# paschalidoud/raynet

Hardware: AMD Instinct MI355X
Metric: rays/sec (whole node) at 5 views x 64 depths x 128^3 voxels (higher is better)
Workload: dtype f32

## Files before the change

include/raynet_hip.h:

```cpp
#ifndef RAYNET_HIP_H
#define RAYNET_HIP_H

#include <stdint.h>

#ifdef __cplusplus
extern "C" {
#endif

typedef enum {
    RN_OK = 0,
    RN_ERR_INVALID = -1,
    RN_ERR_HIP = -2,
    RN_ERR_NO_DEVICE = -3,
    RN_ERR_STATE = -4
} rn_status;

typedef struct {
    int32_t M;
    int32_t D;
    int32_t N;
    int32_t F;
    int32_t H;
    int32_t W;
    int32_t padding;
// ... 160 lines not shown
    RN_RUN_DEPTH_RANGE = 16
} rn_run_phase;
int rn_scene_run(rn_ctx *ctx, const rn_scene_plan *plan, int32_t phases, int32_t iteration,
                 int32_t image, void *stream);

int rn_stitch_rows(rn_ctx *ctx, int64_t n, const float *rows, const int32_t *index, float *out,
                   void *stream);

typedef enum {
    RN_K_TRAVERSE = 1,
    RN_K_SWEEP_MAP = 2,
    RN_K_BP = 3,
    RN_K_DEPTH = 4,
    RN_K_ACC = 5,
    RN_K_OTHER = 6,
    RN_K_SCATTER = 7
} rn_kernel_id;
int rn_prof_begin(rn_ctx *ctx, int32_t capacity);
int rn_prof_select(rn_ctx *ctx, uint32_t kernel_mask);
int rn_prof_end(rn_ctx *ctx, int32_t *count, int32_t *kernel_ids_host, int32_t *n_rays_host,
                float *ms_host);
int rn_prof_offsets(rn_ctx *ctx, float *start_ms_host);

int rn_selftest_arith(rn_ctx *ctx, int32_t n, const float *a, float *out, void *stream);
int rn_selftest_quotient(rn_ctx *ctx, int32_t n, const float *x, const float *d, float *out,
                         void *stream);

int rn_selftest_feature_offsets(rn_ctx *ctx, int32_t n, const float *P, const float *ray_start,
                                const float *ray_end, int32_t *out, void *stream);

int rn_selftest_mapping(rn_ctx *ctx, int32_t n, const float *a, const float *b, const float *t,
                        float *out, void *stream);


int rn_plane_weights(rn_ctx *ctx, int32_t n, const int32_t *rvi, const int32_t *rvc,
                     const float *ray_start, const float *ray_end, int32_t *left, float *c1,
                     float *c2, void *stream);

int rn_train_bp_sweep(rn_ctx *ctx, int32_t n, const float *Sr, const int32_t *rvi,
                      const int32_t *rvc, const float *acc_in, const float *msgs_in,
                      float *acc_out, float *msgs_out, void *stream);
int rn_train_depth(rn_ctx *ctx, int32_t n, const float *Sr, const int32_t *rvi,
                   const int32_t *rvc, const float *acc, const float *msgs, float *S_new,
                   void *stream);

int rn_train_bp_sweep_bwd(rn_ctx *ctx, int32_t n, const float *Sr, const int32_t *rvi,
                          const int32_t *rvc, const float *acc_in, const float *msgs_in,
                          const float *g_msgs_out, const float *g_acc_out, float *g_Sr,
                          float *g_acc_in, float *g_msgs_in, void *stream);

int rn_train_depth_bwd(rn_ctx *ctx, int32_t n, const float *Sr, const int32_t *rvi,
                       const int32_t *rvc, const float *acc, const float *msgs,
                       const float *g_S_new, float *g_Sr, float *g_acc, float *g_msgs,
                       void *stream);


int rn_depthmap_points(rn_ctx *ctx, int32_t H, int32_t W, const double *P_pinv,
                       const double *camera_center, const float *depth_map, double *points,
                       void *stream);

int rn_consistency_tau(rn_ctx *ctx, int32_t n, int32_t H, int32_t W, int32_t first,
                       const double *points, const double *P, const double *camera_center,
                       const float *depth_map, double *tau, void *stream);

int rn_nearest_neighbors(rn_ctx *ctx, int32_t n_ref, const float *ref_xyzw, int32_t n_query,
                         const float *query_xyzw, float *dist, int32_t *idx, void *stream);
// ... 47 lines not shown
```

raynet_amd/_lib.py:

```python
import ctypes
import os
import subprocess

_HERE = os.path.dirname(os.path.abspath(__file__))
CSRC = os.path.join(_HERE, "csrc")
ENV_LIB = os.environ.get("RAYNET_HIP_LIB") or None
LIB_PATH = ENV_LIB or os.path.join(CSRC, "libraynet_hip.so")
HEADER = os.path.join(os.path.dirname(_HERE), "include", "raynet_hip.h")

HIPCC_FLAGS = [
    "--offload-arch=gfx950", "-O3", "-std=c++17",
    "-ffp-contract=off",
    "-munsafe-fp-atomics",
    "-Wno-unused-value", "-fPIC", "-shared",
]

RN_OK = 0
STATUS = {0: "RN_OK", -1: "RN_ERR_INVALID", -2: "RN_ERR_HIP", -3: "RN_ERR_NO_DEVICE",
          -4: "RN_ERR_STATE"}


class RaynetHipError(RuntimeError):
    pass

# ... 108 lines not shown
    "rn_scene_bp_sweep_fixed": [_P, _I, _P, _P, _P, _P, _P, _P, _I, _I, _P],
    "rn_acc_combine_fixed": [_P, _P, _F, _P, _P],
    "rn_acc_combine_fixed_range": [_P, _P, _L, _F, _P, _P],
    "rn_acc_combine": [_P, _P, _F, _P, _P],
    "rn_acc_reduce_local": [_P, _P, _P, _P],
    "rn_acc_add_prior": [_P, _P, _F, _P],
    "rn_scene_depth": [_P, _I, _P, _P, _P, _P, _P, _P, _I, _P, _P, _P],
    "rn_prof_begin": [_P, _I],
    "rn_prof_select": [_P, ctypes.c_uint32],
    "rn_prof_end": [_P, ctypes.POINTER(_I), _P, _P, _P],
    "rn_plane_weights": [_P, _I, _P, _P, _P, _P, _P, _P, _P, _P],
    "rn_train_bp_sweep": [_P, _I, _P, _P, _P, _P, _P, _P, _P, _P],
    "rn_train_depth": [_P, _I, _P, _P, _P, _P, _P, _P, _P],
    "rn_train_bp_sweep_bwd": [_P, _I] + [_P] * 11,
    "rn_train_depth_bwd": [_P, _I] + [_P] * 10,
    "rn_depthmap_points": [_P, _I, _I, _P, _P, _P, _P, _P],
    "rn_consistency_tau": [_P, _I, _I, _I, _I, _P, _P, _P, _P, _P, _P],
    "rn_nearest_neighbors": [_P, _I, _P, _I, _P, _P, _P, _P],
    "rn_mesh_keys": [_P, _I, _P, _P, _P, _P],
    "rn_mesh_build": [_P, _I, _P, _P, _P, _P, _P, ctypes.POINTER(_I), _P],
    "rn_mesh_raycast": [_P, _I, _P, _P, _P, _P, _P, _P, _P],
    "rn_mesh_depthmap": [_P, _I, _I, _P, _P, _P, _P, _P, _P],
    "rn_mesh_closest": [_P, _I, _P, _P, _P, _P, _P, _P, _P],
    "rn_mesh_areas": [_P, _I, _P, _P, _P],
    "rn_mesh_sample": [_P, _I, _I, _P, _P, _L, _P, _P, _P],
    "rn_voxel_mask": [_P, _I, _P, _P, _I, _I, _I, _P, _P, _P],
    "rn_thin_keys": [_P, _I, _P, _D, _D, _D, _D, _L, _P, _P, _P, _P],
    "rn_thin_round": [_P, _I, _P, _I, _P, _P, _P, _P, _D, _P, _P, _P],
    "rn_prof_offsets": [_P, _P],
    "rn_selftest_arith": [_P, _I, _P, _P, _P],
    "rn_selftest_quotient": [_P, _I, _P, _P, _P, _P],
    "rn_selftest_mapping": [_P, _I, _P, _P, _P, _P, _P],
    "rn_selftest_feature_offsets": [_P, _I, _P, _P, _P, _P, _P],
    "rn_timer_start": [_P, _P],
    "rn_timer_stop": [_P, _P, ctypes.POINTER(_F)],
}

_lib = None


def load():
    global _lib
    if _lib is not None:
        return _lib
    if not os.path.exists(LIB_PATH):
        raise RaynetHipError(
            "%s is missing: run `python -c 'import __graft_entry__ as g; g.build()'` "
            "(raynet_amd has no CPU fallback)" % LIB_PATH)
    import torch
    lib = ctypes.CDLL(LIB_PATH)
    for name, argtypes in SIGNATURES.items():
        fn = getattr(lib, name)
        fn.argtypes = argtypes
        fn.restype = ctypes.c_int
    lib.rn_destroy.restype = None
    lib.rn_last_error.restype = ctypes.c_char_p
    lib.rn_version.restype = ctypes.c_char_p
    lib.rn_acc_size.restype = ctypes.c_int64
    lib.rn_slab_boxes_size.restype = ctypes.c_int64
    _lib = lib
    return lib
```

raynet_amd/csrc/raynet_hip.hip:

```cpp
#include "raynet_kernels.h"

#include <cstdarg>
#include <cstdio>
#include <cstdlib>
#include <iterator>
#include <type_traits>
#include <utility>
#include <vector>

#include "../../include/raynet_hip.h"
#include "raynet_box_policy.h"

using namespace rn;

namespace {

constexpr int BLOCK = 256;
constexpr int RAY_BLOCK = 256;
constexpr int WAVES_PER_BLOCK = BLOCK / WAVE;
constexpr int SWEEP_BLOCK = 256;
constexpr int SWEEP_WAVES = SWEEP_BLOCK / WAVE;
constexpr int NXCD = 8;

constexpr int XCD_CHUNK_SWEEP = 2048 * 64 / 256;
// ... 66 lines not shown
__global__ __launch_bounds__(BLOCK) void k_selftest_arith(int n, const float *__restrict__ a,
                                                          float *out) {
    const int i = blockIdx.x * BLOCK + threadIdx.x;
    if (i >= n) return;
    out[i] = roundf(a[i]);
    out[(size_t)n + i] = round_half_away(a[i]);
}
__global__ __launch_bounds__(BLOCK) void k_selftest_quotient(int n, const float *__restrict__ x,
                                                             const float *__restrict__ d,
                                                             float *out) {
    const int i = blockIdx.x * BLOCK + threadIdx.x;
    if (i >= n) return;
    bool sure;
    const float rd = __builtin_amdgcn_rcpf(d[i]);
    const float fast = round_quotient_fast(x[i], rd, sure);
    sure = sure && reciprocal_is_normal(rd);
    out[i] = round_half_away(x[i] / d[i]);
    out[(size_t)n + i] = fast;
    out[2 * (size_t)n + i] = sure ? 1.0f : 0.0f;
}
__global__ __launch_bounds__(BLOCK) void k_selftest_offsets(Params p, int n,
                                                            const float *__restrict__ P,
                                                            const float *__restrict__ starts,
                                                            const float *__restrict__ ends,
                                                            int32_t *out) {
    int lane;
    const int r = ray_of_wave(n, lane);
    if (r < 0) return;
    float s[3], e[3];
    for (int i = 0; i < 3; i++) {
        s[i] = starts[3 * r + i];
        e[i] = ends[3 * r + i];
    }
    const float pad_shift = (float)(p.padding - (p.padding - 1) / 2);
    for (int base = 0; base < p.D; base += WAVE) {
        const int k = min(base + lane, p.D - 1);
        float point[3];
        plane_point(s, e, k, p.D, point);
        for (int v = 0; v < p.N; v++) {
            const int generic = feature_offset(p, P + 12 * v, point) / p.F;
            const int coop = feature_offset_bytes<7>(p, P + 12 * v, point, pad_shift) >> 7;
            if (base + lane < p.D) {
                int32_t *o = out + (((size_t)r * p.N + v) * p.D + k) * 2;
                o[0] = generic;
                o[1] = coop;
            }
        }
    }
}
__global__ __launch_bounds__(BLOCK) void k_selftest_mapping(Params p, int n,
                                                            const float *__restrict__ a,
                                                            const float *__restrict__ b,
                                                            const float *__restrict__ t,
                                                            float *out) {
    extern __shared__ float pos[];
    for (int i = threadIdx.x; i <= p.D; i += BLOCK) pos[i] = 0.0f + i * p.plane_step;
    __syncthreads();
    const int i = blockIdx.x * BLOCK + threadIdx.x;
    if (i >= n) return;
    const float y = 1.0f / b[i];
    out[i] = a[i] / b[i];
    out[(size_t)n + i] = markstein_div(a[i], b[i], y);
    out[2 * (size_t)n + i] = markstein_ok(b[i]) && markstein_ok_dividend(a[i]) ? 1.0f : 0.0f;
    const float tc = clampf(t[i], 1e-4f, 1 - 1e-4f);
    out[3 * (size_t)n + i] = (float)plane_index_walk(tc, p.D, p.plane_step);
    out[4 * (size_t)n + i] = (float)plane_index_from_table(pos, tc, p.D);
}
template <bool TO_GRID>
__global__ void k_acc_regrid(Params p, const float *__restrict__ src, float *dst) {
    const int64_t G = (int64_t)p.gx * p.gy * p.gz;
    for (int64_t i = blockIdx.x * (int64_t)blockDim.x + threadIdx.x; i < G;
         i += (int64_t)gridDim.x * blockDim.x) {
        const int z = (int)(i % p.gz), y = (int)((i / p.gz) % p.gy), x = (int)(i / ((int64_t)p.gz * p.gy));
        const int64_t b = ((((int64_t)(x >> 2) * p.nby + (y >> 2)) * p.nbz + (z >> 2)) << 6) |
                          ((x & 3) << 4) | ((y & 3) << 2) | (z & 3);
        if (TO_GRID) dst[i] = src[b];
        else dst[b] = src[i];
    }
}
__global__ void k_stitch_rows(int64_t n, const float *__restrict__ rows,
                              const int32_t *__restrict__ index, float *out) {
    const int64_t n4 = n >> 2;
    for (int64_t i = blockIdx.x * (int64_t)blockDim.x + threadIdx.x; i < n4;
         i += (int64_t)gridDim.x * blockDim.x) {
        const int4 ix = reinterpret_cast<const int4 *>(index)[i];
        reinterpret_cast<float4 *>(out)[i] = make_float4(rows[ix.x], rows[ix.y], rows[ix.z], rows[ix.w]);
    }
    if (blockIdx.x == 0 && threadIdx.x < (n & 3)) {
        const int64_t i = (n4 << 2) + threadIdx.x;
        out[i] = rows[index[i]];
    }
}
__global__ void k_add_scalar(float *a, int64_t n, float v) {
    for (int64_t i = blockIdx.x * (int64_t)blockDim.x + threadIdx.x; i < n;
         i += (int64_t)gridDim.x * blockDim.x)
        a[i] = v + a[i];
}

#include "raynet_prepare.inl"
// ... 798 lines not shown
    RN_OPEN(ctx, n, all_set(a, out));
    hipLaunchKernelGGL(k_selftest_arith, dim3(thread_blocks(n)), dim3(BLOCK), 0, S(stream), n, a, out);
    RN_LAUNCH_CHECK(ctx);
    return RN_OK;
}

int rn_selftest_quotient(rn_ctx *ctx, int32_t n, const float *x, const float *d, float *out,
                         void *stream) {
    RN_OPEN(ctx, n, all_set(x, d, out));
    hipLaunchKernelGGL(k_selftest_quotient, dim3(thread_blocks(n)), dim3(BLOCK), 0, S(stream), n, x,
                       d, out);
    RN_LAUNCH_CHECK(ctx);
    return RN_OK;
}

int rn_selftest_feature_offsets(rn_ctx *ctx, int32_t n, const float *P, const float *ray_start,
                                const float *ray_end, int32_t *out, void *stream) {
    RN_OPEN(ctx, n, all_set(P, ray_start, ray_end, out));
    hipLaunchKernelGGL(k_selftest_offsets, dim3(ray_blocks(n)), dim3(BLOCK), 0, S(stream), ctx->p, n,
                       P, ray_start, ray_end, out);
    RN_LAUNCH_CHECK(ctx);
    return RN_OK;
}

int rn_selftest_mapping(rn_ctx *ctx, int32_t n, const float *a, const float *b, const float *t,
                        float *out, void *stream) {
    RN_OPEN(ctx, n, all_set(a, b, t, out));
    hipLaunchKernelGGL(k_selftest_mapping, dim3(thread_blocks(n)), dim3(BLOCK),
                       sizeof(float) * (ctx->p.D + 1), S(stream), ctx->p, n, a, b, t, out);
    RN_LAUNCH_CHECK(ctx);
    return RN_OK;
}

int rn_prof_offsets(rn_ctx *ctx, float *start_ms_host) {
    if (!ctx || !start_ms_host) return fail(ctx, RN_ERR_INVALID, "bad argument");
    for (int i = 0; i < ctx->prof_n; i++)
        RN_HIP(ctx, hipEventElapsedTime(start_ms_host + i, ctx->prof_ev[0], ctx->prof_ev[2 * i]));
    return RN_OK;
}


int rn_timer_start(rn_ctx *ctx, void *stream) {
    if (!ctx) return RN_ERR_INVALID;
    RN_HIP(ctx, hipEventRecord(ctx->ev0, S(stream)));
    return RN_OK;
}

int rn_timer_stop(rn_ctx *ctx, void *stream, float *ms_out) {
    if (!ctx || !ms_out) return RN_ERR_INVALID;
    RN_HIP(ctx, hipEventRecord(ctx->ev1, S(stream)));
    RN_HIP(ctx, hipEventSynchronize(ctx->ev1));
    RN_HIP(ctx, hipEventElapsedTime(ms_out, ctx->ev0, ctx->ev1));
    return RN_OK;
}

}

#include "raynet_train.inl"

#include "raynet_eval.inl"

#include "raynet_mesh.inl"

#include "raynet_filters.inl"
```

raynet_amd/csrc/raynet_kernels.h:

```cpp
#pragma once
#include <hip/hip_runtime.h>
#include <float.h>
#include <stdint.h>

namespace rn {

constexpr int WAVE = 64;
constexpr int MAX_VIEWS = 16;

typedef float float2v __attribute__((ext_vector_type(2)));
typedef float float4v __attribute__((ext_vector_type(4)));

struct Params {
    int M, D, N, F, H, W, padding;
    int gx, gy, gz;
    int nby, nbz;
    int Hf, Wf;
    float plane_step;
    float bbox[6];
};

struct FeatureViews {
    const float *v[MAX_VIEWS];
};
// ... 55 lines not shown
__device__ __forceinline__ float wave_sum(float x) {
    RN_WAVE_REDUCE("v_add_f32_dpp", x);
    return lane63(x);
}
__device__ __forceinline__ float wave_max(float x) {
    RN_WAVE_REDUCE("v_max_f32_dpp", x);
    return lane63(x);
}
__device__ __forceinline__ int wave_max_i(int x) {
    RN_WAVE_REDUCE("v_max_i32_dpp", x);
    return lane63i(x);
}
__device__ __forceinline__ int wave_min_i(int x) {
    RN_WAVE_REDUCE("v_min_i32_dpp", x);
    return lane63i(x);
}
__device__ __forceinline__ int uniform(int x) { return __builtin_amdgcn_readfirstlane(x); }
__device__ __forceinline__ void wave_sync() {
    __builtin_amdgcn_fence(__ATOMIC_ACQ_REL, "wavefront");
    __builtin_amdgcn_wave_barrier();
}

__device__ __forceinline__ float clampf(float x, float a, float b) {
    return __builtin_amdgcn_fmed3f(x, a, b);
}

__device__ __forceinline__ float round_half_away(float x) {
    return __builtin_truncf(x + __builtin_copysignf(0x1.fffffep-2f, x));
}

__device__ __forceinline__ bool reciprocal_is_normal(float rcp_n) {
    return __builtin_amdgcn_classf(rcp_n, 0x108);
}
__device__ __forceinline__ float round_quotient_fast(float x, float rcp_n, bool &sure) {
    const float q = x * rcp_n;
    const float r = __builtin_rintf(q);
    sure = __builtin_fabsf(q - r) < __builtin_fmaf(__builtin_fabsf(q), -0x1p-21f, 0.5f);
    return r;
}

__device__ __forceinline__ void sample_in_bbox(const Params &p, int ray_idx,
                                               const float *__restrict__ P_inv,
                                               const float *__restrict__ cc, float s[3],
                                               float e[3]) {
    const float px = (float)(ray_idx / p.H);
    const float py = (float)(ray_idx % p.H);
    double o[4];
#pragma unroll
    for (int r = 0; r < 4; r++) {
        double a = 0.0;
        a += (double)(P_inv[3 * r + 0] * px);
        a += (double)(P_inv[3 * r + 1] * py);
        a += (double)P_inv[3 * r + 2] * 1.0;
        o[r] = a;
    }
    float dir[3];
#pragma unroll
    for (int i = 0; i < 3; i++) dir[i] = (float)(o[i] / o[3] - (double)cc[i]);
    float t_near = -INFINITY, t_far = INFINITY;
#pragma unroll
    for (int i = 0; i < 3; i++) {
        const float t1 = (float)(((double)p.bbox[i] - (double)cc[i]) / (double)dir[i]);
        const float t2 = (float)(((double)p.bbox[3 + i] - (double)cc[i]) / (double)dir[i]);
        t_near = fmaxf(fminf(t1, t2), t_near);
        t_far = fminf(fmaxf(t1, t2), t_far);
    }
    const float near_mask = (fabsf(t_near) < fabsf(t_far)) ? 1.0f : 0.0f;
    const float tn = t_near * near_mask + t_far * (1 - near_mask);
    const float tf = (1 - near_mask) * t_near + near_mask * t_far;
#pragma unroll
    for (int i = 0; i < 3; i++) {
        s[i] = cc[i] + tn * dir[i];
        e[i] = cc[i] + tf * dir[i];
    }
}

__device__ __forceinline__ int feature_offset(const Params &p, const float *__restrict__ Pv,
                                              const float point[3]) {
    float x = 0.0f, y = 0.0f, n = 0.0f;
    x += Pv[0] * point[0]; x += Pv[1] * point[1]; x += Pv[2] * point[2]; x += Pv[3] * 1;
    y += Pv[4] * point[0]; y += Pv[5] * point[1]; y += Pv[6] * point[2]; y += Pv[7] * 1;
    n += Pv[8] * point[0]; n += Pv[9] * point[1]; n += Pv[10] * point[2]; n += Pv[11] * 1;
    x = x / n;
    y = y / n;
    const int half = (p.padding - 1) / 2;
    int fx = (int)(roundf(x) + p.padding - half);
    int fy = (int)(roundf(y) + p.padding - half);
    fx = min(max(fx, 0), p.W);
    fy = min(max(fy, 0), p.H);
    if (fx == 0 || fy == 0) fx = fy = 0;
    return (fy * p.Wf + fx) * p.F;
}

__device__ __forceinline__ void project_fast(const float *__restrict__ Pv, const float point[3],
                                             float &x, float &y, float &n, float &rx, float &ry,
                                             unsigned long long &sure) {
    x = Pv[0] * point[0]; y = Pv[4] * point[0]; n = 0.0f;
    x += Pv[1] * point[1]; x += Pv[2] * point[2]; x += Pv[3] * 1;
    y += Pv[5] * point[1]; y += Pv[6] * point[2]; y += Pv[7] * 1;
    n += Pv[8] * point[0]; n += Pv[9] * point[1]; n += Pv[10] * point[2]; n += Pv[11] * 1;
    const float rn = __builtin_amdgcn_rcpf(n);
    bool sure_x, sure_y;
    rx = round_quotient_fast(x, rn, sure_x);
    ry = round_quotient_fast(y, rn, sure_y);
    unsigned long long normal_rcp;
    asm("v_cmp_class_f32_e64 %0, %1, %2" : "=s"(normal_rcp) : "v"(rn), "v"(0x108));
    sure = __builtin_amdgcn_ballot_w64(sure_x) & __builtin_amdgcn_ballot_w64(sure_y) & normal_rcp;
}
__device__ __forceinline__ void project_ieee(float x, float y, float n, float &rx, float &ry) {
    rx = round_half_away(x / n);
    ry = round_half_away(y / n);
}
template <int LOG2_VEC_BYTES>
__device__ __forceinline__ int project_offset(const Params &p, float rx, float ry, float pad_shift) {
    rx += pad_shift;
    ry += pad_shift;
    const unsigned fx = (unsigned)(int)__builtin_amdgcn_fmed3f(rx, 0.0f, (float)p.W);
    const unsigned fy = (unsigned)(int)__builtin_amdgcn_fmed3f(ry, 0.0f, (float)p.H);
    const unsigned off = (__umul24(fy, (unsigned)p.Wf) + fx) << LOG2_VEC_BYTES;
    return min(fx, fy) == 0u ? 0 : (int)off;
}
template <int LOG2_VEC_BYTES>
__device__ __forceinline__ int feature_offset_bytes(const Params &p,
                                                    const float *__restrict__ Pv,
                                                    const float point[3], float pad_shift) {
    float x, y, n, rx, ry;
    unsigned long long sure;
    project_fast(Pv, point, x, y, n, rx, ry, sure);
    if (sure != __builtin_amdgcn_read_exec())
        project_ieee(x, y, n, rx, ry);
    return project_offset<LOG2_VEC_BYTES>(p, rx, ry, pad_shift);
}

__device__ __forceinline__ void plane_point(const float s[3], const float e[3], int k, int D,
                                            float point[3]) {
#pragma unroll
    for (int a = 0; a < 3; a++) point[a] = s[a] + k * (e[a] - s[a]) / (D - 1);
}

__device__ __forceinline__ void sweep_generic(const Params &p, const FeatureViews &fv,
                                              const float *const *__restrict__ tbl,
                                              const float *__restrict__ P, const float s[3],
                                              const float e[3], int lane, float *Sl) {
    const int pairs = (p.N * (p.N - 1)) / 2;
    for (int base = 0; base < p.D; base += WAVE) {
        const int k = base + lane;
        if (k < p.D) {
            float point[3];
            plane_point(s, e, k, p.D, point);
            float acc = 0.0f;
            for (int i = 0; i < p.N; i++) {
                const float *fi = (tbl ? tbl[i] : fv.v[i]) + feature_offset(p, P + 12 * i, point);
                for (int j = i + 1; j < p.N; j++) {
                    const float *fj =
                        (tbl ? tbl[j] : fv.v[j]) + feature_offset(p, P + 12 * j, point);
                    float dot = 0.0f;
                    for (int f = 0; f < p.F; f++) dot += fi[f] * fj[f];
                    acc += dot;
                }
            }
            Sl[k] = acc / pairs;
        }
    }
}

constexpr int SWEEP_V4 = 1;
constexpr int SWEEP_UNROLL2_MAX_VIEWS = 6;
#define RN_ADD_DPP(OUT, MOVED, STAY, CTRL)                                                   \
    asm("s_nop 1\n\tv_add_f32_dpp %0, %1, %2 " CTRL " row_mask:0xf bank_mask:0xf"           \
        : "=v"(OUT) : "v"(MOVED), "v"(STAY))
#define RN_DPP_XOR1 "quad_perm:[1,0,3,2]"
#define RN_DPP_XOR2 "quad_perm:[2,3,0,1]"
#define RN_DPP_MIRROR8 "row_half_mirror"

template <int NV, int V4, bool REF_HELD = false>
__device__ __forceinline__ float sweep_round(const float *const (&vbase)[NV], const int (&offb)[NV],
                                             int src, unsigned part_bytes,
                                             const float2v (&ref)[2 * V4]) {
    float2v f2[NV][2 * V4];
#pragma unroll
    for (int v = 0; v < NV; v++) {
        if (REF_HELD && v == 0) {
#pragma unroll
            for (int c = 0; c < 2 * V4; c++) f2[0][c] = ref[c];
            continue;
        }
        const unsigned ob = (unsigned)__shfl(offb[v], src) + part_bytes;
        typedef const __attribute__((address_space(1))) char *gptr;
        typedef const __attribute__((address_space(1))) float4v *gptr4;
#pragma unroll
        for (int q = 0; q < V4; q++) {
            const float4v f = *(gptr4)((gptr)vbase[v] + ob + 16u * q);
            f2[v][2 * q] = float2v{f.x, f.y};
            f2[v][2 * q + 1] = float2v{f.z, f.w};
        }
    }
    float acc;
    {
#pragma clang fp contract(fast)
        float2v run[2 * V4], a2[2 * V4];
#pragma unroll
        for (int c = 0; c < 2 * V4; c++) {
            run[c] = f2[0][c];
            a2[c] = float2v{0.f, 0.f};
        }
#pragma unroll
        for (int j = 1; j < NV; j++) {
#pragma unroll
            for (int c = 0; c < 2 * V4; c++) {
                a2[c] = run[c] * f2[j][c] + a2[c];
                if (j + 1 < NV) run[c] += f2[j][c];
            }
        }
        float2v t = a2[0];
#pragma unroll
        for (int c = 1; c < 2 * V4; c++) t += a2[c];
        acc = t.x + t.y;
    }
    return acc;
}

template <int NV, int LPS, int V4, bool REF_HELD, int RPW, bool PARTIAL>
__device__ __forceinline__ float sweep_rounds(const float *const (&vbase)[NV], const int (&offb)[NV],
                                              int sub, int part, unsigned part_bytes,
                                              const float2v (&ref)[RPW][2 * V4], int live, int nrays,
                                              int &mine_round) {
    constexpr int SPL = WAVE / LPS;
    constexpr int DPAD = WAVE / RPW;
    static_assert(DPAD % (2 * SPL) == 0 || LPS != 8, "a pair of load rounds stays within one ray");
    float mine = 0.0f;
    if (LPS == 8 && NV <= SWEEP_UNROLL2_MAX_VIEWS) {
        const bool odd = (part ^ (part >> 2)) & 1;
        mine_round = (part & ~1) | (int)odd;
#pragma unroll
        for (int t = 0; t < LPS / 2; t++) {
            const int first = (2 * t) * SPL;
            if (PARTIAL && (first % DPAD >= live || first / DPAD >= nrays)) continue;
            const float2v(&rf)[2 * V4] = ref[RPW == 1 ? 0 : first / DPAD];
            const float a0 = sweep_round<NV, V4, REF_HELD>(vbase, offb, first + sub, part_bytes, rf);
            const float a1 = sweep_round<NV, V4, REF_HELD>(vbase, offb, first + SPL + sub, part_bytes, rf);
            const float stay = odd ? a1 : a0, moved = odd ? a0 : a1;
            float r;
            RN_ADD_DPP(r, moved, stay, RN_DPP_XOR1);
            RN_ADD_DPP(r, r, r, RN_DPP_XOR2);
            RN_ADD_DPP(r, r, r, RN_DPP_MIRROR8);
            if ((part >> 1) == t) mine = r;
        }
    } else {
        static_assert(LPS <= 8, "sweep_coop folds at most 8 lanes per plane");
        mine_round = part;
#pragma unroll
        for (int it = 0; it < LPS; it++) {
            const int first = it * SPL;
            if (PARTIAL && (first % DPAD >= live || first / DPAD >= nrays)) continue;
            float acc = sweep_round<NV, V4, REF_HELD>(vbase, offb, first + sub, part_bytes,
                                                      ref[RPW == 1 ? 0 : first / DPAD]);
            if (LPS >= 2) RN_ADD_DPP(acc, acc, acc, RN_DPP_XOR1);
            if (LPS >= 4) RN_ADD_DPP(acc, acc, acc, RN_DPP_XOR2);
            if (LPS >= 8) RN_ADD_DPP(acc, acc, acc, RN_DPP_MIRROR8);
            if (part == it) mine = acc;
        }
    }
    return mine;
}

template <int NV, int LPS, bool FAST = false, int RPW = 1>
__device__ __forceinline__ void sweep_coop(const Params &p, const FeatureViews &fv,
                                           const float *const *__restrict__ tbl,
                                           const float *__restrict__ P, const float s[3],
                                           const float e[3], int lane, float *Sl, int nrays = 1) {
    constexpr int SPL = WAVE / LPS;
    constexpr int V4 = SWEEP_V4;
    constexpr int DPAD = WAVE / RPW;
    const float *vbase[NV];
#pragma unroll
    for (int v = 0; v < NV; v++) vbase[v] = tbl ? tbl[v] : fv.v[v];
    const int sub = lane / LPS;
    const int part = lane % LPS;
    const unsigned part_bytes = (16u * V4) * (unsigned)part;
    const int pairs = (NV * (NV - 1)) / 2;
    constexpr int LOG2_VEC_BYTES = LPS * V4 == 8 ? 7 : LPS * V4 == 4 ? 6 : LPS * V4 == 2 ? 5 : 4;
    static_assert((16 * V4 * LPS) == (1 << LOG2_VEC_BYTES), "vector bytes must be a power of two");
    const float pad_shift = (float)(p.padding - (p.padding - 1) / 2);
    const int q_lane = RPW == 1 ? 0 : lane / DPAD;
    for (int base = 0; base < (RPW == 1 ? p.D : 1); base += WAVE) {
        int offb[NV];
        {
            const int k = min(RPW == 1 ? base + lane : lane % DPAD, p.D - 1);
            float point[3];
            plane_point(s, e, k, p.D, point);
#pragma unroll
            for (int v = 0; v < NV; v++)
                offb[v] = feature_offset_bytes<LOG2_VEC_BYTES>(p, P + 12 * v, point, pad_shift);
        }
        int off0[RPW];
#pragma unroll
        for (int q = 0; q < RPW; q++) off0[q] = __builtin_amdgcn_readlane(offb[0], q * DPAD);
        int off0_mine = off0[0];
#pragma unroll
        for (int q = 1; q < RPW; q++) off0_mine = q_lane == q ? off0[q] : off0_mine;
        const bool ref_held = __all(offb[0] == off0_mine);
        float2v ref[RPW][2 * V4];
#pragma unroll
        for (int q = 0; q < RPW; q++)
#pragma unroll
            for (int c = 0; c < 2 * V4; c++) ref[q][c] = float2v{0.f, 0.f};
        if (ref_held) {
            typedef const __attribute__((address_space(1))) char *gptr;
            typedef const __attribute__((address_space(1))) float4v *gptr4;
#pragma unroll
            for (int q = 0; q < RPW; q++)
#pragma unroll
                for (int c = 0; c < V4; c++) {
                    const float4v f = *(gptr4)((gptr)vbase[0] + (unsigned)off0[q] + part_bytes + 16u * c);
                    ref[q][2 * c] = float2v{f.x, f.y};
                    ref[q][2 * c + 1] = float2v{f.z, f.w};
                }
        }
        float mine = 0.0f;
        int mine_round;
        const int live = RPW == 1 ? p.D - base : p.D;
        const bool full = live >= DPAD && nrays == RPW;
        if (ref_held && full)
            mine = sweep_rounds<NV, LPS, V4, true, RPW, false>(vbase, offb, sub, part, part_bytes, ref, live, nrays, mine_round);
        else if (ref_held)
            mine = sweep_rounds<NV, LPS, V4, true, RPW, true>(vbase, offb, sub, part, part_bytes, ref, live, nrays, mine_round);
        else
            mine = sweep_rounds<NV, LPS, V4, false, RPW, true>(vbase, offb, sub, part, part_bytes, ref, live, nrays, mine_round);
        const int j = mine_round * SPL + sub;
        const int k = RPW == 1 ? base + j : j % DPAD;
        const int q = RPW == 1 ? 0 : j / DPAD;
        if (k < p.D && q < nrays) Sl[q * p.D + k] = FAST ? mine * (1.0f / pairs) : mine / pairs;
    }
}

#define RN_GROUP_REDUCE16(OP, X)                                                 \
    RN_SCAN_STEP(OP, X, "quad_perm:[1,0,3,2] row_mask:0xf bank_mask:0xf");       \
    RN_SCAN_STEP(OP, X, "quad_perm:[2,3,0,1] row_mask:0xf bank_mask:0xf");       \
    RN_SCAN_STEP(OP, X, "row_half_mirror row_mask:0xf bank_mask:0xf");           \
// ... 6 lines not shown
    return lane < 32 ? lo : hi;
}
template <int G>
__device__ __forceinline__ float group_max(float x, int lane) {
    static_assert(G == 16 || G == 32, "groups of 16 or 32 lanes");
    RN_GROUP_REDUCE16("v_max_f32_dpp", x);
    if (G == 32) RN_SCAN_STEP("v_max_f32_dpp", x, "row_bcast:15 row_mask:0xa bank_mask:0xf");
    return group_pick<G>(x, lane);
}
template <int G>
__device__ __forceinline__ float group_sum(float x, int lane) {
    static_assert(G == 16 || G == 32, "groups of 16 or 32 lanes");
    RN_GROUP_REDUCE16("v_add_f32_dpp", x);
    if (G == 32) RN_SCAN_STEP("v_add_f32_dpp", x, "row_bcast:15 row_mask:0xa bank_mask:0xf");
    return group_pick<G>(x, lane);
}

template <bool FAST>
__device__ __forceinline__ float vdiv(float a, float b) {
    return FAST ? a * __builtin_amdgcn_rcpf(b) : a / b;
}
__device__ __forceinline__ float exp_nonpos(float x) {
    const float log2e_hi = 0x1.715476p+0f, log2e_lo = 0x1.4ae0bep-26f;
    const float ph = x * log2e_hi;
    float pl = __builtin_fmaf(x, log2e_hi, -ph);
    pl = __builtin_fmaf(x, log2e_lo, pl);
    const float e = __builtin_rintf(ph);
    const float a = (ph - e) + pl;
    const float r = __builtin_amdgcn_ldexpf(__builtin_amdgcn_exp2f(a), (int)e);
    return x < -0x1.9d1da00000000p+6f ? 0.0f : r;
}
template <bool FAST = false>
__device__ __forceinline__ void softmax_column(int D, int lane, float *Sl) {
    float mx = -INFINITY;
    for (int k = lane; k < D; k += WAVE) mx = fmaxf(mx, Sl[k]);
    mx = wave_max(mx);
    float sum = 0.0f;
    for (int k = lane; k < D; k += WAVE) {
        const float d = Sl[k] - mx;
#if !defined(RN_EXACT_OCC_EXP) && !defined(RN_EXACT_SOFTMAX_EXP)
        const float v = FAST ? __builtin_amdgcn_exp2f(d * 0x1.715476p+0f)
                             : (d <= 0.0f ? exp_nonpos(d) : expf(d));
#else
        const float v = d <= 0.0f ? exp_nonpos(d) : expf(d);
#endif
        Sl[k] = v;
        sum += v;
    }
    sum = wave_sum(sum);
    for (int k = lane; k < D; k += WAVE) Sl[k] = vdiv<FAST>(Sl[k], sum);
}

template <bool FAST, int RPW>
__device__ __forceinline__ void softmax_columns(int D, int lane, float *Sl) {
    constexpr int DPAD = WAVE / RPW;
    const int k = lane % DPAD;
    float *x = Sl + (lane / DPAD) * D + k;
    const bool mine = k < D;
    const float mx = group_max<DPAD>(mine ? *x : -INFINITY, lane);
    float v = 0.0f;
    if (mine) {
        const float d = *x - mx;
#if !defined(RN_EXACT_OCC_EXP) && !defined(RN_EXACT_SOFTMAX_EXP)
        v = FAST ? __builtin_amdgcn_exp2f(d * 0x1.715476p+0f) : (d <= 0.0f ? exp_nonpos(d) : expf(d));
#else
        v = d <= 0.0f ? exp_nonpos(d) : expf(d);
// ... 17 lines not shown
        z = row[3 * i + 2];
    }
}
__device__ __forceinline__ int pack_voxel(int x, int y, int z) {
    return (x << 20) | (y << 10) | z;
}

constexpr int SLAB_BOX_STEPS = 16;
__host__ __device__ __forceinline__ int slab_box_count(int M) {
    return (M + SLAB_BOX_STEPS - 1) / SLAB_BOX_STEPS;
}

__device__ __forceinline__ float markstein_div(float a, float b, float y) {
    const float q0 = a * y;
    const float r = __builtin_fmaf(-b, q0, a);
    return __builtin_fmaf(r, y, q0);
}
__device__ __forceinline__ bool markstein_ok(float b) {
    return b >= 0x1p-60f && b <= 0x1p60f;
}
__device__ __forceinline__ bool markstein_ok_dividend(float a) {
    return __builtin_fabsf(a) < 0x1p60f;
}
__device__ __forceinline__ int plane_index_from_table(const float *pos, float t, int D) {
    const int a = max((int)(t * (D - 1)), 1);
    return (a - 1) + (pos[a] < t ? 1 : 0) + (pos[a + 1] < t ? 1 : 0);
}
__device__ __forceinline__ int plane_index_walk(float t, int D, float step) {
    int L = max(0, (int)(t * (D - 1)) - 1);
    while ((t - (0.0f + L * step) > 0) && (t - (0.0f + (L + 1) * step) > 0)) L++;
    return L;
}

template <bool PACKED, bool FAST = false, bool STAGED = false, bool TABLE = false>
__device__ __forceinline__ float map_planes_to_voxels(const Params &p,
                                                      const float *__restrict__ axes,
                                                      const int32_t *__restrict__ vrow,
                                                      int count, const float s[3],
                                                      const float e[3], const float *Sl,
                                                      float *vals, int lane, int n_staged = 0,
                                                      const float *pos = nullptr) {
    const float eps = 1e-4f;
    float ray[3], ray_norm = 0.0f;
#pragma unroll
    for (int i = 0; i < 3; i++) ray[i] = e[i] - s[i];
#pragma unroll
    for (int i = 0; i < 3; i++) ray_norm += ray[i] * ray[i];
    const float step = p.plane_step;
    const bool div_ok = TABLE && markstein_ok(ray_norm);
    const float rcp_norm = TABLE ? 1.0f / ray_norm : 0.0f;
    int carry = 0;
    float total = 0.0f;
    for (int base = 0; base < count; base += WAVE) {
        const int i = base + lane;
        const bool valid = i < count;
        int L = 0;
        float t = 0.0f;
        if (valid) {
            int x, y, z;
            if (PACKED && STAGED) {
                const int v = __builtin_bit_cast(int, vals[i]);
                x = v >> 20;
                y = (v >> 10) & 1023;
                z = v & 1023;
            } else {
                load_voxel<PACKED>(vrow, i, x, y, z);
            }
            float sum = 0.0f;
            float vd = axes[x];
            vd -= s[0];
            sum += ray[0] * vd;
            vd = axes[p.gx + y];
            vd -= s[1];
            sum += ray[1] * vd;
            vd = axes[p.gx + p.gy + z];
            vd -= s[2];
            sum += ray[2] * vd;
            if (TABLE) {
                float q;
                if (div_ok && __all(markstein_ok_dividend(sum))) q = markstein_div(sum, ray_norm, rcp_norm);
                else q = sum / ray_norm;
                t = clampf(q, eps, 1 - eps);
                L = plane_index_from_table(pos, t, p.D);
            } else {
                t = clampf(sum / ray_norm, eps, 1 - eps);
                L = plane_index_walk(t, p.D, step);
            }
        }
        int left = max(wave_scan_max(valid ? L : 0), carry);
        carry = lane63i(left);
        float val = 0.0f;
        if (valid) {
            const int right = left + 1;
            float left_d = fabsf(t - (TABLE ? pos[left] : 0.0f + left * step));
            float right_d = fabsf(t - (TABLE ? pos[right] : 0.0f + right * step));
            const float c1 = 1.0f - vdiv<FAST>(left_d, left_d + right_d);
            const float c2 = 1.0f - vdiv<FAST>(right_d, left_d + right_d);
            val = c1 * Sl[left] + c2 * Sl[right];
            vals[i] = val;
        }
        total += val;
    }
    return wave_sum(total);
}
// ... 29 lines not shown
```

raynet_amd/hip_implementations/context.py:

```python
import ctypes

import numpy as np
import torch

from .. import _lib


def _stream():
    return ctypes.c_void_p(torch.cuda.current_stream().cuda_stream)


def _ptr(t):
    if t is None:
        return ctypes.c_void_p(0)
    if not t.is_cuda or not t.is_contiguous():
        raise ValueError("the C ABI takes contiguous CUDA tensors (got %s, %s)" % (
            "cuda" if t.is_cuda else "cpu", "contiguous" if t.is_contiguous() else "strided"))
    return ctypes.c_void_p(t.data_ptr())


def _chk(t, dtype, min_numel=0, name="tensor", optional=False, align=4):
    if t is None:
        if optional:
            return t
# ... 391 lines not shown
        self._check(self.lib.rn_prof_select(self._h, mask))
        self._prof_cap = capacity
        self.prof_active = True
        self._check(self.lib.rn_prof_begin(self._h, capacity))

    def prof_end(self):
        cap = self._prof_cap
        self.prof_active = False
        ids = (ctypes.c_int32 * cap)()
        rays = (ctypes.c_int32 * cap)()
        ms = (ctypes.c_float * cap)()
        n = ctypes.c_int32()
        self._check(self.lib.rn_prof_end(self._h, ctypes.byref(n), ids, rays, ms))
        starts = (ctypes.c_float * cap)()
        self._check(self.lib.rn_prof_offsets(self._h, starts))
        self.prof_starts = [float(starts[i]) for i in range(n.value)]
        return [(self.KERNEL_NAMES.get(ids[i], str(ids[i])), int(rays[i]), float(ms[i]))
                for i in range(n.value)]

    def selftest_arith(self, a, out):
        self._check(self.lib.rn_selftest_arith(self._h, a.numel(), _ptr(a), _ptr(out), _stream()))

    def selftest_quotient(self, x, d, out):
        self._check(self.lib.rn_selftest_quotient(self._h, x.numel(), _ptr(x), _ptr(d), _ptr(out),
                                                  _stream()))

    def selftest_feature_offsets(self, P, starts, ends, out):
        self._check(self.lib.rn_selftest_feature_offsets(self._h, len(starts), _ptr(P), _ptr(starts),
                                                         _ptr(ends), _ptr(out), _stream()))

    def selftest_mapping(self, a, b, t, out):
        self._check(self.lib.rn_selftest_mapping(self._h, a.numel(), _ptr(a), _ptr(b), _ptr(t),
                                                 _ptr(out), _stream()))

    def fill_f32(self, t, value):
        self._check(self.lib.rn_fill_f32(self._h, _ptr(t), t.numel(), float(value), _stream()))

    def fill_i32(self, t, value):
        self._check(self.lib.rn_fill_i32(self._h, _ptr(t), t.numel(), int(value), _stream()))

    def sample_rays(self, ray_idxs, P_inv, center, starts, ends):
        self._check(self.lib.rn_sample_rays(self._h, len(ray_idxs), _ptr(ray_idxs), _ptr(P_inv),
                                            _ptr(center), _ptr(starts), _ptr(ends), _stream()))

    def sample_points(self, ray_idxs, P_inv, center, points):
        self._check(self.lib.rn_sample_points(self._h, len(ray_idxs), _ptr(ray_idxs), _ptr(P_inv),
                                              _ptr(center), _ptr(points), _stream()))

    def compute_similarities(self, features, P, starts, ends, S):
        self._check(self.lib.rn_compute_similarities(self._h, len(starts), _ptr(features), _ptr(P),
                                                     _ptr(starts), _ptr(ends), _ptr(S), _stream()))

    def voxel_traversal(self, starts, ends, rvi, rvc):
        self._check(self.lib.rn_voxel_traversal(self._h, len(starts), _ptr(starts), _ptr(ends),
                                                _ptr(rvi), _ptr(rvc), _stream()))

    def planes_to_voxels(self, rvi, rvc, starts, ends, S, S_new):
        self._check(self.lib.rn_planes_to_voxels(self._h, len(rvc), _ptr(rvi), _ptr(rvc),
                                                 _ptr(starts), _ptr(ends), _ptr(S), _ptr(S_new),
                                                 _stream()))

    def bp_sweep(self, S, rvi, rvc, acc_in, msgs_in, acc_out, msgs_out):
        self._check(self.lib.rn_bp_sweep(self._h, len(rvc), _ptr(S), _ptr(rvi), _ptr(rvc),
                                         _ptr(acc_in), _ptr(msgs_in), _ptr(acc_out),
                                         _ptr(msgs_out), _stream()))

# ... 210 lines not shown
```

Measured before the change: 235.3 million.

## Micro-optimize projection, plane points, sweep shuffles and small-D softmax

Bundles several arithmetic micro-optimizations in the sweep path. Plane points use a reciprocal-based Markstein division when a guard holds, and projection uses packed float2 math with an integer-pad mad24 offset. Lane shuffles become direct ds_bpermute, the unused zero-init of ref registers is dropped, and a single-pass softmax is added for D<=WAVE. Selftest kernels are added to check bit-exactness, since the fast paths risk subtle rounding differences.

```diff
diff --git a/include/raynet_hip.h b/include/raynet_hip.h
--- a/include/raynet_hip.h
+++ b/include/raynet_hip.h
@@ -216,6 +216,14 @@
 int rn_selftest_mapping(rn_ctx *ctx, int32_t n, const float *a, const float *b, const float *t,
                         float *out, void *stream);
 
+int rn_selftest_plane_points(rn_ctx *ctx, int32_t n, const float *ray_start, const float *ray_end,
+                             float *out, int32_t *ok, void *stream);
+int rn_selftest_projection(rn_ctx *ctx, int32_t n, const float *P, const float *points,
+                           int32_t *out, void *stream);
+int rn_selftest_mapping_tail(rn_ctx *ctx, int32_t n, const int32_t *vox, const int32_t *rvc,
+                             const float *ray_start, const float *ray_end, const float *Sp,
+                             float *out, void *stream);
+
 
 int rn_plane_weights(rn_ctx *ctx, int32_t n, const int32_t *rvi, const int32_t *rvc,
                      const float *ray_start, const float *ray_end, int32_t *left, float *c1,
diff --git a/raynet_amd/_lib.py b/raynet_amd/_lib.py
--- a/raynet_amd/_lib.py
+++ b/raynet_amd/_lib.py
@@ -164,6 +164,9 @@
     "rn_selftest_quotient": [_P, _I, _P, _P, _P, _P],
     "rn_selftest_mapping": [_P, _I, _P, _P, _P, _P, _P],
     "rn_selftest_feature_offsets": [_P, _I, _P, _P, _P, _P, _P],
+    "rn_selftest_plane_points": [_P, _I, _P, _P, _P, _P, _P],
+    "rn_selftest_projection": [_P, _I, _P, _P, _P, _P],
+    "rn_selftest_mapping_tail": [_P, _I, _P, _P, _P, _P, _P, _P, _P],
     "rn_timer_start": [_P, _P],
     "rn_timer_stop": [_P, _P, ctypes.POINTER(_F)],
 }
diff --git a/raynet_amd/csrc/raynet_hip.hip b/raynet_amd/csrc/raynet_hip.hip
--- a/raynet_amd/csrc/raynet_hip.hip
+++ b/raynet_amd/csrc/raynet_hip.hip
@@ -122,14 +122,14 @@
         s[i] = starts[3 * r + i];
         e[i] = ends[3 * r + i];
     }
-    const float pad_shift = (float)(p.padding - (p.padding - 1) / 2);
+    const int pad = p.padding - (p.padding - 1) / 2;
     for (int base = 0; base < p.D; base += WAVE) {
         const int k = min(base + lane, p.D - 1);
         float point[3];
         plane_point(s, e, k, p.D, point);
         for (int v = 0; v < p.N; v++) {
             const int generic = feature_offset(p, P + 12 * v, point) / p.F;
-            const int coop = feature_offset_bytes<7>(p, P + 12 * v, point, pad_shift) >> 7;
+            const int coop = feature_offset_bytes<7>(p, P + 12 * v, point, pad) >> 7;
             if (base + lane < p.D) {
                 int32_t *o = out + (((size_t)r * p.N + v) * p.D + k) * 2;
                 o[0] = generic;
@@ -155,6 +155,87 @@
     const float tc = clampf(t[i], 1e-4f, 1 - 1e-4f);
     out[3 * (size_t)n + i] = (float)plane_index_walk(tc, p.D, p.plane_step);
     out[4 * (size_t)n + i] = (float)plane_index_from_table(pos, tc, p.D);
+}
+__global__ __launch_bounds__(BLOCK) void k_selftest_plane_points(Params p, int n,
+                                                                 const float *__restrict__ starts,
+                                                                 const float *__restrict__ ends,
+                                                                 float *out, int32_t *ok) {
+    int lane;
+    const int r = ray_of_wave(n, lane);
+    if (r < 0) return;
+    float s[3], e[3];
+    for (int i = 0; i < 3; i++) {
+        s[i] = starts[3 * r + i];
+        e[i] = ends[3 * r + i];
+    }
+    const bool uni = plane_quotients_ok<true>(s, e, p.D), per_lane = plane_quotients_ok<false>(s, e, p.D);
+    if (lane == 0) ok[r] = (uni ? 1 : 0) | (per_lane ? 2 : 0);
+    for (int k = lane; k < p.D; k += WAVE) {
+        float exact[3], fast[3];
+        plane_point(s, e, k, p.D, exact);
+        plane_point_fast(s, e, k, p.D, p.plane_step, fast);
+        float *o = out + ((size_t)r * p.D + k) * 6;
+        for (int i = 0; i < 3; i++) {
+            o[i] = exact[i];
+            o[3 + i] = fast[i];
+        }
+    }
+}
+__global__ __launch_bounds__(BLOCK) void k_selftest_projection(Params p, int n,
+                                                               const float *__restrict__ P,
+                                                               const float *__restrict__ points,
+                                                               int32_t *out) {
+    const int t = blockIdx.x * BLOCK + threadIdx.x;
+    const int i = min(t, n - 1);
+    const float *Pv = P + 12 * (size_t)i;
+    const float point[3] = {points[3 * (size_t)i], points[3 * (size_t)i + 1], points[3 * (size_t)i + 2]};
+    const int pad = p.padding - (p.padding - 1) / 2;
+    float x, y, nn, rx, ry, ex, ey;
+    unsigned long long sure;
+    project_fast(Pv, point, x, y, nn, rx, ry, sure);
+    project_ieee(x, y, nn, ex, ey);
+    const int lane = threadIdx.x & (WAVE - 1);
+    if (t >= n) return;
+    out[4 * (size_t)i] = feature_offset(p, Pv, point) / p.F;
+    out[4 * (size_t)i + 1] = project_offset<7>(p, ex, ey, pad) >> 7;
+    out[4 * (size_t)i + 2] = project_offset<7>(p, rx, ry, pad) >> 7;
+    out[4 * (size_t)i + 3] = (int)((sure >> lane) & 1);
+}
+__global__ __launch_bounds__(WAVE) void k_selftest_mapping_tail(Params p, const float *__restrict__ axes_g,
+                                                                const int32_t *__restrict__ vox,
+                                                                const int32_t *__restrict__ rvc,
+                                                                const float *__restrict__ starts,
+                                                                const float *__restrict__ ends,
+                                                                const float *__restrict__ S, float *out) {
+    extern __shared__ __attribute__((aligned(16))) float smem[];
+    const int naxes = p.gx + p.gy + p.gz;
+    float *axes = smem;
+    float *pos = smem + ((naxes + 3) & ~3);
+    float *Sl = pos + ((p.D + 4) & ~3);
+    float *vals = Sl + p.D;
+    const int lane = threadIdx.x, r = blockIdx.x;
+    for (int i = lane; i < naxes; i += WAVE) axes[i] = axes_g[i];
+    for (int i = lane; i <= p.D; i += WAVE) pos[i] = 0.0f + i * p.plane_step;
+    for (int k = lane; k < p.D; k += WAVE) Sl[k] = S[(size_t)r * p.D + k];
+    float s[3], e[3];
+    for (int i = 0; i < 3; i++) {
+        s[i] = starts[3 * r + i];
+        e[i] = ends[3 * r + i];
+    }
+    const int count = min(rvc[r], p.M);
+    const int32_t *vrow = vox + (size_t)r * p.M;
+    for (int side = 0; side < 2; side++) {
+        for (int i = lane; i < count; i += WAVE) vals[i] = __builtin_bit_cast(float, vrow[i]);
+        __syncthreads();
+        const float sum = side == 0
+            ? map_planes_to_voxels<true, true, true, true, true>(p, axes, vrow, count, s, e, Sl, vals, lane, count, pos)
+            : map_planes_to_voxels<true, true, true, true, false>(p, axes, vrow, count, s, e, Sl, vals, lane, count, pos);
+        __syncthreads();
+        float *o = out + ((size_t)r * 2 + side) * (p.M + 1);
+        for (int i = lane; i < count; i += WAVE) o[i] = vals[i];
+        if (lane == 0) o[p.M] = sum;
+        __syncthreads();
+    }
 }
 template <bool TO_GRID>
 __global__ void k_acc_regrid(Params p, const float *__restrict__ src, float *dst) {
@@ -1019,6 +1100,40 @@
     return RN_OK;
 }
 
+int rn_selftest_plane_points(rn_ctx *ctx, int32_t n, const float *ray_start, const float *ray_end,
+                             float *out, int32_t *ok, void *stream) {
+    RN_OPEN(ctx, n, all_set(ray_start, ray_end, out, ok));
+    hipLaunchKernelGGL(k_selftest_plane_points, dim3(ray_blocks(n)), dim3(BLOCK), 0, S(stream),
+                       ctx->p, n, ray_start, ray_end, out, ok);
+    RN_LAUNCH_CHECK(ctx);
+    return RN_OK;
+}
+
+int rn_selftest_projection(rn_ctx *ctx, int32_t n, const float *P, const float *points,
+                           int32_t *out, void *stream) {
+    RN_OPEN(ctx, n, all_set(P, points, out));
+    if (ctx->p.F != 32) return fail(ctx, RN_ERR_INVALID, "rn_selftest_projection: F must be 32");
+    hipLaunchKernelGGL(k_selftest_projection, dim3(thread_blocks(n)), dim3(BLOCK), 0, S(stream),
+                       ctx->p, n, P, points, out);
+    RN_LAUNCH_CHECK(ctx);
+    return RN_OK;
+}
+
+int rn_selftest_mapping_tail(rn_ctx *ctx, int32_t n, const int32_t *vox, const int32_t *rvc,
+                             const float *ray_start, const float *ray_end, const float *Sp,
+                             float *out, void *stream) {
+    RN_OPEN(ctx, n, all_set(vox, rvc, ray_start, ray_end, Sp, out));
+    if (!ctx->axes) return fail(ctx, RN_ERR_STATE, "rn_selftest_mapping_tail: no voxel grid set");
+    const Params &p = ctx->p;
+    const size_t lds = sizeof(float) * ((size_t)((p.gx + p.gy + p.gz + 3) & ~3) +
+                                        (size_t)((p.D + 4) & ~3) + p.D + p.M);
+    if (lds > 64 * 1024) return fail(ctx, RN_ERR_INVALID, "rn_selftest_mapping_tail: shape too large");
+    hipLaunchKernelGGL(k_selftest_mapping_tail, dim3(n), dim3(WAVE), lds, S(stream), p, ctx->axes,
+                       vox, rvc, ray_start, ray_end, Sp, out);
+    RN_LAUNCH_CHECK(ctx);
+    return RN_OK;
+}
+
 int rn_prof_offsets(rn_ctx *ctx, float *start_ms_host) {
     if (!ctx || !start_ms_host) return fail(ctx, RN_ERR_INVALID, "bad argument");
     for (int i = 0; i < ctx->prof_n; i++)
diff --git a/raynet_amd/csrc/raynet_kernels.h b/raynet_amd/csrc/raynet_kernels.h
--- a/raynet_amd/csrc/raynet_kernels.h
+++ b/raynet_amd/csrc/raynet_kernels.h
@@ -111,10 +111,15 @@
 __device__ __forceinline__ bool reciprocal_is_normal(float rcp_n) {
     return __builtin_amdgcn_classf(rcp_n, 0x108);
 }
+__device__ __forceinline__ float quotient_margin(float q) {
+    float b;
+    asm("v_fma_f32 %0, |%1|, %2, 0.5" : "=v"(b) : "v"(q), "s"(-0x1p-21f));
+    return b;
+}
 __device__ __forceinline__ float round_quotient_fast(float x, float rcp_n, bool &sure) {
     const float q = x * rcp_n;
     const float r = __builtin_rintf(q);
-    sure = __builtin_fabsf(q - r) < __builtin_fmaf(__builtin_fabsf(q), -0x1p-21f, 0.5f);
+    sure = __builtin_fabsf(q - r) < quotient_margin(q);
     return r;
 }
 
@@ -174,14 +179,20 @@
 __device__ __forceinline__ void project_fast(const float *__restrict__ Pv, const float point[3],
                                              float &x, float &y, float &n, float &rx, float &ry,
                                              unsigned long long &sure) {
-    x = Pv[0] * point[0]; y = Pv[4] * point[0]; n = 0.0f;
-    x += Pv[1] * point[1]; x += Pv[2] * point[2]; x += Pv[3] * 1;
-    y += Pv[5] * point[1]; y += Pv[6] * point[2]; y += Pv[7] * 1;
+    float2v xy = float2v{Pv[0], Pv[4]} * point[0];
+    n = 0.0f;
+    xy += float2v{Pv[1], Pv[5]} * point[1];
+    xy += float2v{Pv[2], Pv[6]} * point[2];
+    xy += float2v{Pv[3], Pv[7]} * 1;
     n += Pv[8] * point[0]; n += Pv[9] * point[1]; n += Pv[10] * point[2]; n += Pv[11] * 1;
+    x = xy.x; y = xy.y;
     const float rn = __builtin_amdgcn_rcpf(n);
-    bool sure_x, sure_y;
-    rx = round_quotient_fast(x, rn, sure_x);
-    ry = round_quotient_fast(y, rn, sure_y);
+    const float2v q = xy * rn;
+    rx = __builtin_rintf(q.x);
+    ry = __builtin_rintf(q.y);
+    const float2v d = q - float2v{rx, ry};
+    const bool sure_x = __builtin_fabsf(d.x) < quotient_margin(q.x);
+    const bool sure_y = __builtin_fabsf(d.y) < quotient_margin(q.y);
     unsigned long long normal_rcp;
     asm("v_cmp_class_f32_e64 %0, %1, %2" : "=s"(normal_rcp) : "v"(rn), "v"(0x108));
     sure = __builtin_amdgcn_ballot_w64(sure_x) & __builtin_amdgcn_ballot_w64(sure_y) & normal_rcp;
@@ -191,30 +202,54 @@
     ry = round_half_away(y / n);
 }
 template <int LOG2_VEC_BYTES>
-__device__ __forceinline__ int project_offset(const Params &p, float rx, float ry, float pad_shift) {
-    rx += pad_shift;
-    ry += pad_shift;
-    const unsigned fx = (unsigned)(int)__builtin_amdgcn_fmed3f(rx, 0.0f, (float)p.W);
-    const unsigned fy = (unsigned)(int)__builtin_amdgcn_fmed3f(ry, 0.0f, (float)p.H);
-    const unsigned off = (__umul24(fy, (unsigned)p.Wf) + fx) << LOG2_VEC_BYTES;
-    return min(fx, fy) == 0u ? 0 : (int)off;
+__device__ __forceinline__ int project_offset(const Params &p, float rx, float ry, int pad) {
+    const int fx = (int)__builtin_amdgcn_fmed3f(rx, (float)-pad, (float)(p.W - pad));
+    const int fy = (int)__builtin_amdgcn_fmed3f(ry, (float)-pad, (float)(p.H - pad));
+    const unsigned origin = (unsigned)(pad * p.Wf + pad) << LOG2_VEC_BYTES;
+    int row;
+    asm("v_mad_i32_i24 %0, %1, %2, %3" : "=v"(row) : "v"(fy), "s"(p.Wf), "v"(fx));
+    const unsigned off = ((unsigned)row << LOG2_VEC_BYTES) + origin;
+    return min(fx, fy) == -pad ? 0 : (int)off;
 }
 template <int LOG2_VEC_BYTES>
 __device__ __forceinline__ int feature_offset_bytes(const Params &p,
                                                     const float *__restrict__ Pv,
-                                                    const float point[3], float pad_shift) {
+                                                    const float point[3], int pad) {
     float x, y, n, rx, ry;
     unsigned long long sure;
     project_fast(Pv, point, x, y, n, rx, ry, sure);
     if (sure != __builtin_amdgcn_read_exec())
         project_ieee(x, y, n, rx, ry);
-    return project_offset<LOG2_VEC_BYTES>(p, rx, ry, pad_shift);
+    return project_offset<LOG2_VEC_BYTES>(p, rx, ry, pad);
 }
 
 __device__ __forceinline__ void plane_point(const float s[3], const float e[3], int k, int D,
                                             float point[3]) {
 #pragma unroll
     for (int a = 0; a < 3; a++) point[a] = s[a] + k * (e[a] - s[a]) / (D - 1);
+}
+
+__device__ __forceinline__ float markstein_div(float a, float b, float y);
+template <bool UNIFORM>
+__device__ __forceinline__ bool plane_quotients_ok(const float s[3], const float e[3], int D) {
+    bool ok = D >= 2 && D <= 4096;
+#pragma unroll
+    for (int a = 0; a < 3; a++) {
+        int d = __builtin_bit_cast(int, e[a] - s[a]), sb = __builtin_bit_cast(int, s[a]);
+        if (UNIFORM) {
+            d = uniform(d);
+            sb = uniform(sb);
+        }
+        const unsigned m = (unsigned)d & 0x7fffffffu;
+        ok = ok && (m == 0u || m - 0x21800000u < 0x57800000u - 0x21800000u) && (unsigned)sb != 0x80000000u;
+    }
+    return UNIFORM ? ok : (bool)__all(ok);
+}
+__device__ __forceinline__ void plane_point_fast(const float s[3], const float e[3], int k, int D,
+                                                 float rcp_dm1, float point[3]) {
+    const float b = (float)(D - 1);
+#pragma unroll
+    for (int a = 0; a < 3; a++) point[a] = s[a] + markstein_div(k * (e[a] - s[a]), b, rcp_dm1);
 }
 
 __device__ __forceinline__ void sweep_generic(const Params &p, const FeatureViews &fv,
@@ -254,7 +289,7 @@
 
 template <int NV, int V4, bool REF_HELD = false>
 __device__ __forceinline__ float sweep_round(const float *const (&vbase)[NV], const int (&offb)[NV],
-                                             int src, unsigned part_bytes,
+                                             int first, int sub4, unsigned part_bytes,
                                              const float2v (&ref)[2 * V4]) {
     float2v f2[NV][2 * V4];
 #pragma unroll
@@ -264,7 +299,7 @@
             for (int c = 0; c < 2 * V4; c++) f2[0][c] = ref[c];
             continue;
         }
-        const unsigned ob = (unsigned)__shfl(offb[v], src) + part_bytes;
+        const unsigned ob = (unsigned)__builtin_amdgcn_ds_bpermute(sub4 + 4 * first, offb[v]) + part_bytes;
         typedef const __attribute__((address_space(1))) char *gptr;
         typedef const __attribute__((address_space(1))) float4v *gptr4;
 #pragma unroll
@@ -307,6 +342,7 @@
     constexpr int SPL = WAVE / LPS;
     constexpr int DPAD = WAVE / RPW;
     static_assert(DPAD % (2 * SPL) == 0 || LPS != 8, "a pair of load rounds stays within one ray");
+    const int sub4 = sub << 2;
     float mine = 0.0f;
     if (LPS == 8 && NV <= SWEEP_UNROLL2_MAX_VIEWS) {
         const bool odd = (part ^ (part >> 2)) & 1;
@@ -316,8 +352,8 @@
             const int first = (2 * t) * SPL;
             if (PARTIAL && (first % DPAD >= live || first / DPAD >= nrays)) continue;
             const float2v(&rf)[2 * V4] = ref[RPW == 1 ? 0 : first / DPAD];
-            const float a0 = sweep_round<NV, V4, REF_HELD>(vbase, offb, first + sub, part_bytes, rf);
-            const float a1 = sweep_round<NV, V4, REF_HELD>(vbase, offb, first + SPL + sub, part_bytes, rf);
+            const float a0 = sweep_round<NV, V4, REF_HELD>(vbase, offb, first, sub4, part_bytes, rf);
+            const float a1 = sweep_round<NV, V4, REF_HELD>(vbase, offb, first + SPL, sub4, part_bytes, rf);
             const float stay = odd ? a1 : a0, moved = odd ? a0 : a1;
             float r;
             RN_ADD_DPP(r, moved, stay, RN_DPP_XOR1);
@@ -332,7 +368,7 @@
         for (int it = 0; it < LPS; it++) {
             const int first = it * SPL;
             if (PARTIAL && (first % DPAD >= live || first / DPAD >= nrays)) continue;
-            float acc = sweep_round<NV, V4, REF_HELD>(vbase, offb, first + sub, part_bytes,
+            float acc = sweep_round<NV, V4, REF_HELD>(vbase, offb, first, sub4, part_bytes,
                                                       ref[RPW == 1 ? 0 : first / DPAD]);
             if (LPS >= 2) RN_ADD_DPP(acc, acc, acc, RN_DPP_XOR1);
             if (LPS >= 4) RN_ADD_DPP(acc, acc, acc, RN_DPP_XOR2);
@@ -360,17 +396,19 @@
     const int pairs = (NV * (NV - 1)) / 2;
     constexpr int LOG2_VEC_BYTES = LPS * V4 == 8 ? 7 : LPS * V4 == 4 ? 6 : LPS * V4 == 2 ? 5 : 4;
     static_assert((16 * V4 * LPS) == (1 << LOG2_VEC_BYTES), "vector bytes must be a power of two");
-    const float pad_shift = (float)(p.padding - (p.padding - 1) / 2);
+    const int pad = p.padding - (p.padding - 1) / 2;
     const int q_lane = RPW == 1 ? 0 : lane / DPAD;
+    const bool fast_points = plane_quotients_ok<RPW == 1>(s, e, p.D);
     for (int base = 0; base < (RPW == 1 ? p.D : 1); base += WAVE) {
         int offb[NV];
         {
             const int k = min(RPW == 1 ? base + lane : lane % DPAD, p.D - 1);
             float point[3];
-            plane_point(s, e, k, p.D, point);
+            if (fast_points) plane_point_fast(s, e, k, p.D, p.plane_step, point);
+            else plane_point(s, e, k, p.D, point);
 #pragma unroll
             for (int v = 0; v < NV; v++)
-                offb[v] = feature_offset_bytes<LOG2_VEC_BYTES>(p, P + 12 * v, point, pad_shift);
+                offb[v] = feature_offset_bytes<LOG2_VEC_BYTES>(p, P + 12 * v, point, pad);
         }
         int off0[RPW];
 #pragma unroll
@@ -380,10 +418,6 @@
         for (int q = 1; q < RPW; q++) off0_mine = q_lane == q ? off0[q] : off0_mine;
         const bool ref_held = __all(offb[0] == off0_mine);
         float2v ref[RPW][2 * V4];
-#pragma unroll
-        for (int q = 0; q < RPW; q++)
-#pragma unroll
-            for (int c = 0; c < 2 * V4; c++) ref[q][c] = float2v{0.f, 0.f};
         if (ref_held) {
             typedef const __attribute__((address_space(1))) char *gptr;
             typedef const __attribute__((address_space(1))) float4v *gptr4;
@@ -456,6 +490,26 @@
 }
 template <bool FAST = false>
 __device__ __forceinline__ void softmax_column(int D, int lane, float *Sl) {
+    if (D <= WAVE) {
+        const bool mine = lane < D;
+        float mx = -INFINITY;
+        if (mine) mx = fmaxf(mx, Sl[lane]);
+        mx = wave_max(mx);
+        float sum = 0.0f, v = 0.0f;
+        if (mine) {
+            const float d = Sl[lane] - mx;
+#if !defined(RN_EXACT_OCC_EXP) && !defined(RN_EXACT_SOFTMAX_EXP)
+            v = FAST ? __builtin_amdgcn_exp2f(d * 0x1.715476p+0f)
+                     : (d <= 0.0f ? exp_nonpos(d) : expf(d));
+#else
+            v = d <= 0.0f ? exp_nonpos(d) : expf(d);
+#endif
+            sum += v;
+        }
+        sum = wave_sum(sum);
+        if (mine) Sl[lane] = vdiv<FAST>(v, sum);
+        return;
+    }
     float mx = -INFINITY;
     for (int k = lane; k < D; k += WAVE) mx = fmaxf(mx, Sl[k]);
     mx = wave_max(mx);
@@ -539,7 +593,7 @@
     return L;
 }
 
-template <bool PACKED, bool FAST = false, bool STAGED = false, bool TABLE = false>
+template <bool PACKED, bool FAST = false, bool STAGED = false, bool TABLE = false, bool LITERAL = !TABLE>
 __device__ __forceinline__ float map_planes_to_voxels(const Params &p,
                                                       const float *__restrict__ axes,
                                                       const int32_t *__restrict__ vrow,
@@ -573,10 +627,9 @@
             } else {
                 load_voxel<PACKED>(vrow, i, x, y, z);
             }
-            float sum = 0.0f;
             float vd = axes[x];
             vd -= s[0];
-            sum += ray[0] * vd;
+            float sum = LITERAL ? 0.0f + ray[0] * vd : ray[0] * vd;
             vd = axes[p.gx + y];
             vd -= s[1];
             sum += ray[1] * vd;
diff --git a/raynet_amd/hip_implementations/context.py b/raynet_amd/hip_implementations/context.py
--- a/raynet_amd/hip_implementations/context.py
+++ b/raynet_amd/hip_implementations/context.py
@@ -447,6 +447,19 @@
     def selftest_mapping(self, a, b, t, out):
         self._check(self.lib.rn_selftest_mapping(self._h, a.numel(), _ptr(a), _ptr(b), _ptr(t),
                                                  _ptr(out), _stream()))
+
+    def selftest_plane_points(self, starts, ends, out, ok):
+        self._check(self.lib.rn_selftest_plane_points(self._h, len(starts), _ptr(starts), _ptr(ends),
+                                                      _ptr(out), _ptr(ok), _stream()))
+
+    def selftest_projection(self, P, points, out):
+        self._check(self.lib.rn_selftest_projection(self._h, len(points), _ptr(P), _ptr(points),
+                                                    _ptr(out), _stream()))
+
+    def selftest_mapping_tail(self, vox, rvc, starts, ends, S, out):
+        self._check(self.lib.rn_selftest_mapping_tail(self._h, len(rvc), _ptr(vox), _ptr(rvc),
+                                                      _ptr(starts), _ptr(ends), _ptr(S), _ptr(out),
+                                                      _stream()))
 
     def fill_f32(self, t, value):
         self._check(self.lib.rn_fill_f32(self._h, _ptr(t), t.numel(), float(value), _stream()))
```

Result: no change. 234.9 million (-0.2%).
